# ahcorde/visualSLAM_Android

Hardware: AMD Instinct MI355X
Metric: frames/sec (TrackFrame+local BA) on 640×480 synthetic, 1/2/4/8 GPU (higher is better)
Workload: dtype f64

## Files before the change

### visualslam_android_amd/csrc/track.hip

```cpp
#include "vslam_internal.h"
#include "patch_dev.h"
#include "pvs_perm.h"

#define TRK_THREADS 256
#define SORT_CAP 4096
static_assert(SORT_CAP == PVS_SORT_CAP, "a level's list (at most max_points entries) fits the permutation's sort buffer");

template <class T>
DEVFN bool td_project(T& td, int& flags, const double* pos, const Pose& pose, const CamModel& cam, CamProj& pr) {
  flags &= ~TDF_IN_IMAGE;
  double c[3];
  pose_xform(pose, pos, c);
  td.cam[0] = c[0]; td.cam[1] = c[1]; td.cam[2] = c[2];
  if (c[2] < 0.001) return false;
  const double implane[2] = {c[0] / c[2], c[1] / c[2]};
  if (implane[0] * implane[0] + implane[1] * implane[1] > cam.largest_radius * cam.largest_radius) return false;
  pr = cam_project(cam, implane[0], implane[1]);
  td.image[0] = pr.im[0]; td.image[1] = pr.im[1];
  if (pr.invalid) return true;
  if (td.image[0] < 0 || td.image[1] < 0 || td.image[0] > cam.size[0] || td.image[1] > cam.size[1]) return true;
  flags |= TDF_IN_IMAGE;
  return true;
}

// ... 552 lines not shown
  }
  h00 = grp_sum<G>(h00); h01 = grp_sum<G>(h01); h02 = grp_sum<G>(h02);
  h11 = grp_sum<G>(h11); h12 = grp_sum<G>(h12); h22 = grp_sum<G>(h22);
  const double H[9] = {h00, h01, h02, h01, h11, h12, h02, h12, h22};
  double Hinv[9];
  inv3(H, Hinv);
  double sub0 = td.vfound[0], sub1 = td.vfound[1], meanDiff = 0.0;
  bool running = dosub, converged = false;
  for (int it = 0; __any(running); it++) {
    if (it >= nSubPixIts) running = false;
    double cx = 0, cy = 0;
    if (running) {
      cx = level_n_pos(sub0, level); cy = level_n_pos(sub1, level);
      const int xb = (int)(cx > 0.0 ? cx + 0.5 : cx - 0.5), yb = (int)(cy > 0.0 ? cy + 0.5 : cy - 0.5);
      const int b = HALF + 1;
      if (!(xb >= b && yb >= b && xb < cols - b && yb < rows - b)) running = false;
    }
    double p0[Q], p1[Q], p2[Q];
#pragma unroll
    for (int x = 0; x < Q; x++) { p0[x] = 0; p1[x] = 0; p2[x] = 0; }
    if (running && rowok) {
      const double bx = cx - HALF, by = cy - HALF;
      const double dX = bx - floor(bx), dY = by - floor(by);
      const float fTL = (float)((1.0 - dX) * (1.0 - dY)), fTR = (float)((dX) * (1.0 - dY));
      const float fBL = (float)((1.0 - dX) * (dY)), fBR = (float)((dX) * (dY));
      const uint8_t* r0 = img + (size_t)((int)by + sub) * ip + (int)bx + 1;
      const PRow<PS> q0 = load_row<PS>(r0), q1 = load_row<PS>(r0 + ip);
#pragma unroll
      for (int x = 1; x <= Q; x++) {
        const float fPixel = fTL * row_byte(q0, x - 1) + fTR * row_byte(q0, x) + fBL * row_byte(q1, x - 1) + fBR * row_byte(q1, x);
        const double dDiff = (fPixel - (float)row_byte(trow, x)) + meanDiff;
        p0[x - 1] = dDiff * gx[x - 1]; p1[x - 1] = dDiff * gy[x - 1]; p2[x - 1] = dDiff;
      }
    }
    double a0 = 0, a1 = 0, a2 = 0;
#pragma unroll 1
    for (int y = 1; y <= Q; y++) {
      if (sub == y) {
#pragma unroll
        for (int x = 0; x < Q; x++) { a0 += p0[x]; a1 += p1[x]; a2 += p2[x]; }
      }
      const int src = grp * G + y;
      a0 = __shfl(a0, src); a1 = __shfl(a1, src); a2 = __shfl(a2, src);
    }
    if (running) {
      const double u0 = Hinv[0] * a0 + Hinv[1] * a1 + Hinv[2] * a2;
      const double u1 = Hinv[3] * a0 + Hinv[4] * a1 + Hinv[5] * a2;
      const double u2 = Hinv[6] * a0 + Hinv[7] * a1 + Hinv[8] * a2;
      sub0 -= u0 * scale; sub1 -= u1 * scale; meanDiff -= u2;
      if (u0 * u0 + u1 * u1 < 0.03 * 0.03) { converged = true; running = false; }
    }
  }
  if (dosub && lead) {
    if (!converged) tdflags = flags & ~TDF_FOUND;
    else { td.vfound[0] = sub0; td.vfound[1] = sub1; }
  }
  for (int l = 0; l < NLEV; l++) {
    const int c = __popcll(__ballot(dosub && converged && lead && level == l));
    if (lane == 0 && c) atomicAdd(&st->found[l], c);
  }
}

#define SUBPIX_GRID 16
template <int PS, int G>
__global__ __launch_bounds__(64) void k_subpixN(MapDev m, TrackParams tp, SearchArgs a, int stage) {
  int s, bx;
  xcd_stream_block(a.nblk, a.S, s, bx);
  if (s < 0) return;
  TrackerState* st = &m.st[s];
  if (!trk_runs_track_map(m.held, s, st)) return;
  const int nsub = stage == 0 ? st->n_search : st->n_l3;
  for (int blk = bx; blk * (64 / G) < nsub; blk += a.nblk) subpix_block<PS, G>(m, tp, a, st, s, nsub, blk);
}

#define POSE_THREADS 128
#ifdef VSLAM_BA_PROF
__device__ unsigned long long g_pose_prof[16];
#define POSE_STAMP(id) do { if (blockIdx.x == 0 && threadIdx.x == 0) { const unsigned long long t_ = clock64(); g_pose_prof[id] += t_ - g_pose_prof[15]; g_pose_prof[15] = t_; } } while (0)
#else
#define POSE_STAMP(id) do { } while (0)
#endif
#define POSE_WAVES (POSE_THREADS / 64)
#ifndef POSE_ILP
#define POSE_ILP 2
#endif

struct PoseItem {
  double cam[3], image[2], derivs[4], vfound[2], sqrt_inv_noise;
  int flags, idx;
};
struct PoseWs { double* d; int* i; int P; };

DEVFN void item_load(PoseItem& it, const PoseWs& w, int e) {
  it.flags = w.i[e]; it.idx = w.i[w.P + e];
#pragma unroll
  for (int i = 0; i < 3; i++) it.cam[i] = w.d[(0 + i) * w.P + e];
#pragma unroll
  for (int i = 0; i < 2; i++) { it.image[i] = w.d[(3 + i) * w.P + e]; it.vfound[i] = w.d[(9 + i) * w.P + e]; }
#pragma unroll
  for (int i = 0; i < 4; i++) it.derivs[i] = w.d[(5 + i) * w.P + e];
  it.sqrt_inv_noise = w.d[11 * w.P + e];
}
DEVFN void item_store(const PoseItem& it, const PoseWs& w, int e, bool all) {
#pragma unroll
  for (int i = 0; i < 2; i++) w.d[(3 + i) * w.P + e] = it.image[i];
  if (!all) return;
  w.i[e] = it.flags;
#pragma unroll
  for (int i = 0; i < 3; i++) w.d[(0 + i) * w.P + e] = it.cam[i];
#pragma unroll
  for (int i = 0; i < 4; i++) w.d[(5 + i) * w.P + e] = it.derivs[i];
}

#define POSE_CHUNK 32
#define POSE_ENT 27
#define POSE_GRP 8
static_assert(2 * 2 * POSE_CHUNK * POSE_ENT + 2 * POSE_GRP * POSE_ENT + 64 <= SORT_CAP, "two record buffers (and the chain's two groups of read-ahead) in the sort buffer");
static_assert(POSE_THREADS == 128 && POSE_CHUNK == 32 && POSE_GRP % 2 == 0, "wavefront 0 chains, wavefront 1 produces");
static_assert(POSE_THREADS == VSLAM_POSE_WG && SORT_CAP == VSLAM_SELECT_LDS_CAP, "vslam_eval_select / vslam_eval_pose_tail run k_pose's workgroup");

DEVFN void pose_chain_load(double (&v)[POSE_GRP], const double __attribute__((address_space(3)))* p) {
#pragma unroll
  for (int u = 0; u < POSE_GRP; u++) v[u] = p[u * POSE_ENT];
}
DEVFN void pose_chain_add(double& acc, const double (&v)[POSE_GRP]) {
#pragma unroll
  for (int u = 0; u < POSE_GRP; u++) acc += v[u];
}

#ifdef VSLAM_BA_PROF
#define POSE_ACC_PROF_DECL unsigned long long tw_ = 0, tb_ = 0, tl_ = clock64()
#define POSE_ACC_BARRIER() do { const unsigned long long a_ = clock64(); tw_ += a_ - tl_; __syncthreads(); tl_ = clock64(); tb_ += tl_ - a_; } while (0)
#define POSE_ACC_PROF_END() do { if (blockIdx.x == 0 && (threadIdx.x & 63) == 0) { g_pose_prof[10 + 2 * (threadIdx.x >> 6)] += tw_; g_pose_prof[11 + 2 * (threadIdx.x >> 6)] += tb_; } } while (0)
#else
#define POSE_ACC_PROF_DECL do { } while (0)
#define POSE_ACC_BARRIER() __syncthreads()
#define POSE_ACC_PROF_END() do { } while (0)
#endif
#define PAS1 __attribute__((address_space(1)))
#define PAS3 __attribute__((address_space(3)))
__device__ __attribute__((noinline)) double pose_accumulate(const double PAS1* wd, int P, int nf, double wls_prior, bool qint, double sigma2, double PAS3* sortbuf) {
  const int lane = threadIdx.x & 63;
  nf = __builtin_amdgcn_readfirstlane(nf); P = __builtin_amdgcn_readfirstlane(P);
  const int nchunks = (nf + POSE_CHUNK - 1) / POSE_CHUNK;
  constexpr int BUF = 2 * POSE_CHUNK * POSE_ENT;
  POSE_ACC_PROF_DECL;
  double acc = 0.0;
  if (lane == 0 || lane == 6 || lane == 11 || lane == 15 || lane == 18 || lane == 20) acc = 0.0 + wls_prior;
  if (__builtin_amdgcn_readfirstlane(threadIdx.x >> 6) == 1) {
    const int row = lane & 1, pm = lane >> 1;
    struct Item { double cam[3], image[2], vfound[2], da, db, sqrt_inv_noise; };
#define POSE_ITEM_LOADS 10
    auto gld = [&](double& dst, int comp, int e) { asm volatile("global_load_dwordx2 %0, %1, off" : "=v"(dst) : "v"(wd + (size_t)comp * P + e)); };
    auto load_chunk = [&](Item& t, int k) {
      int e = k * POSE_CHUNK + pm;
      e = e < nf ? e : nf - 1;
#pragma unroll
      for (int i = 0; i < 3; i++) gld(t.cam[i], i, e);
#pragma unroll
      for (int i = 0; i < 2; i++) { gld(t.image[i], 3 + i, e); gld(t.vfound[i], 9 + i, e); }
      gld(t.da, 5 + 2 * row, e); gld(t.db, 6 + 2 * row, e);
      gld(t.sqrt_inv_noise, 11, e);
    };
#define POSE_WAIT_SET(t, N) asm volatile("s_waitcnt vmcnt(" #N ")" : "+v"(t.cam[0]), "+v"(t.cam[1]), "+v"(t.cam[2]), "+v"(t.image[0]), "+v"(t.image[1]), \
                                         "+v"(t.vfound[0]), "+v"(t.vfound[1]), "+v"(t.da), "+v"(t.db), "+v"(t.sqrt_inv_noise))
    auto produce = [&](const Item& t, int e, double PAS3* buf) {
      double PAS3* dst = buf + lane * POSE_ENT;
      double w = 0.0, err[2] = {0.0, 0.0};
      if (e < nf) {
        err[0] = (t.vfound[0] - t.image[0]) * t.sqrt_inv_noise; err[1] = (t.vfound[1] - t.image[1]) * t.sqrt_inv_noise;
        const double es = err[0] * err[0] + err[1] * err[1];
        w = tukey_weight(es, sigma2);
      }
      if (w == 0.0) {
#pragma unroll
        for (int k = 0; k < POSE_ENT; k++) dst[k] = 0.0;
        return;
      }
      const double ooz = 1.0 / t.cam[2];
      const double c[3] = {t.cam[0], t.cam[1], t.cam[2]};
      double J[6], wJ[6];
#pragma unroll
      for (int m = 0; m < 6; m++) {
        double f0, f1;
        se3_generator_motion(m, c, ooz, f0, f1);
        J[m] = t.sqrt_inv_noise * (t.da * f0 + t.db * f1);
        wJ[m] = w * J[m];
      }
      const double e_ = row ? err[1] : err[0];
      const double mm = qint ? (double)(int)e_ : e_;
      int q = 0;
#pragma unroll
      for (int r = 0; r < 6; r++)
#pragma unroll
        for (int cc = r; cc < 6; cc++) dst[q++] = wJ[r] * J[cc];
#pragma unroll
      for (int k = 0; k < 6; k++) dst[21 + k] = mm * wJ[k];
    };
    Item it0, it1, it2;
    load_chunk(it0, 0); load_chunk(it1, 1); load_chunk(it2, 2);
    POSE_ACC_BARRIER();
    POSE_WAIT_SET(it0, 20);
    produce(it0, pm, sortbuf);
    POSE_ACC_BARRIER();
    auto prod_step = [&](int k, Item& tprod, Item& tload) {
      if (k + 1 < nchunks) {
        load_chunk(tload, k + 3);
        POSE_WAIT_SET(tprod, 20);
        produce(tprod, (k + 1) * POSE_CHUNK + pm, sortbuf + ((k + 1) & 1) * BUF);
      }
      POSE_ACC_BARRIER();
    };
    for (int k = 0; k < nchunks; k += 3) {
      prod_step(k, it1, it0);
      if (k + 1 < nchunks) prod_step(k + 1, it2, it1);
      if (k + 2 < nchunks) prod_step(k + 2, it0, it2);
    }
    asm volatile("s_waitcnt vmcnt(0)" ::: "memory");
  } else {
    POSE_ACC_BARRIER();
    POSE_ACC_BARRIER();
    for (int k = 0; k < nchunks; k++) {
      const int left = nf - k * POSE_CHUNK;
      const int ng = (2 * (left < POSE_CHUNK ? left : POSE_CHUNK) + POSE_GRP - 1) / POSE_GRP;
      constexpr int GSTR = POSE_GRP * POSE_ENT;
      const double PAS3* rp = sortbuf + (k & 1) * BUF + lane;
      double x0[POSE_GRP], x1[POSE_GRP], x2[POSE_GRP];
      pose_chain_load(x0, rp);
      pose_chain_load(x1, rp + GSTR);
      for (int g = 0; g < ng; g += 3) {
        pose_chain_load(x2, rp + (g + 2) * GSTR);
        __builtin_amdgcn_sched_barrier(0);
        pose_chain_add(acc, x0);
        __builtin_amdgcn_sched_barrier(0);
        if (g + 1 >= ng) break;
        pose_chain_load(x0, rp + (g + 3) * GSTR);
        __builtin_amdgcn_sched_barrier(0);
        pose_chain_add(acc, x1);
        __builtin_amdgcn_sched_barrier(0);
        if (g + 2 >= ng) break;
        pose_chain_load(x1, rp + (g + 4) * GSTR);
        __builtin_amdgcn_sched_barrier(0);
        pose_chain_add(acc, x2);
        __builtin_amdgcn_sched_barrier(0);
      }
      POSE_ACC_BARRIER();
    }
  }
  POSE_ACC_PROF_END();
  return acc;
}

__device__ __attribute__((noinline)) void pose_tail(double acc, double PAS3* pose, double PAS3* up) {
  double mu[6];
  wave_pose_solve(acc, mu);
  POSE_STAMP(6);
  wave_pose_apply(mu, pose);
  if ((threadIdx.x & 63) == 0) {
#pragma unroll
    for (int r = 0; r < 6; r++) up[r] = mu[r];
  }
}

DEVFN void calc_pose_update(const PoseWs& ws, MapPointDev* pts, int nf, const TrackParams& tp,
                            double dOverrideSigma, bool bMarkOutliers, double* sortbuf, Pose* pose ,
                            double* up , int* hist , unsigned long long* sel , const unsigned* selmm ) {
  const bool wave0 = __builtin_amdgcn_readfirstlane(threadIdx.x >> 6) == 0;
  if (nf == 0) {
    if (wave0) pose_tail(0.0, (double PAS3*)(double*)pose, (double PAS3*)up);
    __syncthreads();
    return;
  }
  POSE_STAMP(2);
  double sigma2;
  if (dOverrideSigma > 0) sigma2 = dOverrideSigma;
  else {
    const double med = block_radix_select(sortbuf, nf, nf / 2, hist, sel, selmm);
    sigma2 = tukey_sigma_squared(med, (unsigned long)nf);
  }
  POSE_STAMP(3);
  const double acc = pose_accumulate((const double PAS1*)ws.d, ws.P, nf, tp.wls_prior, (tp.quirks & VSLAM_Q_POSE_INT_RESIDUAL) != 0, sigma2, (double PAS3*)sortbuf);
  if (bMarkOutliers) {
    for (int e = threadIdx.x; e < nf; e += POSE_THREADS) {
      const double sn = ws.d[11 * ws.P + e];
      const double e0 = (ws.d[9 * ws.P + e] - ws.d[3 * ws.P + e]) * sn, e1 = (ws.d[10 * ws.P + e] - ws.d[4 * ws.P + e]) * sn;
      MapPointDev* mp = pts + ws.i[ws.P + e];
      if (tukey_weight(e0 * e0 + e1 * e1, sigma2) == 0.0) mp->n_out++; else mp->n_in++;
    }
  }
  POSE_STAMP(4);
  if (wave0) pose_tail(acc, (double PAS3*)(double*)pose, (double PAS3*)up);
  __syncthreads();
}

#ifndef VSLAM_POSE_WAVES
#define VSLAM_POSE_WAVES 2
#endif
__global__ __launch_bounds__(POSE_THREADS) __attribute__((amdgpu_waves_per_eu(VSLAM_POSE_WAVES, VSLAM_POSE_WAVES))) void k_pose(MapDev m, TrackParams tp, int stage) {
  const int s = blockIdx.x;
  TrackerState* st = &m.st[s];
  if (!trk_runs_track_map(m.held, s, st)) return;
  const int P = tp.max_points;
  TrackData* td = m.td + (size_t)s * P;
  MapPointDev* pts = m.pts + (size_t)s * P;
  const int* ilist = m.iter_list + (size_t)s * P;
  __shared__ double sortbuf[SORT_CAP];
  __shared__ double red[2];
  __shared__ double last_up[6];
  __shared__ int gcnt[4 * POSE_WAVES];
  __shared__ __attribute__((aligned(16))) int hist[768];
  __shared__ unsigned long long sel[1];
  __shared__ unsigned selmm[2 * POSE_WAVES];
  __shared__ Pose pose;
  if (threadIdx.x == 0) pose = st->pose_cur;
  if (threadIdx.x < 6) last_up[threadIdx.x] = 0.0;
  const int n = stage == 0 ? st->n_coarse : st->n_iter;
  if (stage == 0) {
    if (n == 0) return;
    const int nFound = st->found[0] + st->found[1] + st->found[2] + st->found[3];
    if (nFound < tp.coarse_min) return;
  }
#ifdef VSLAM_BA_PROF
  if (blockIdx.x == 0 && threadIdx.x == 0) g_pose_prof[15] = clock64();
#endif
  const PoseWs ws = {m.pose_ws + (size_t)s * POSE_WS_COMPS * P, m.pose_wsi + (size_t)s * 2 * P, P};
  const int lane = threadIdx.x & 63, wave = threadIdx.x >> 6;
  constexpr int POSE_GB = 4;
  int nf = 0;
  for (int e0 = 0; e0 < n; e0 += POSE_GB * POSE_THREADS) {
    int idx[POSE_GB], fl[POSE_GB]; bool fnd[POSE_GB]; unsigned long long bm[POSE_GB]; double v[POSE_GB][12];
#pragma unroll
    for (int u = 0; u < POSE_GB; u++) { const int e = e0 + u * POSE_THREADS + threadIdx.x; idx[u] = ilist[e < n ? e : n - 1]; }
#pragma unroll
    for (int u = 0; u < POSE_GB; u++) {
      const int e = e0 + u * POSE_THREADS + threadIdx.x;
      fl[u] = m.pt_flags[(size_t)s * P + idx[u]];
      fnd[u] = e < n && (fl[u] & TDF_FOUND);
    }
#pragma unroll
    for (int u = 0; u < POSE_GB; u++) {
      const TrackData& t = td[idx[u]];
      for (int i = 0; i < 3; i++) v[u][i] = t.cam[i];
      for (int i = 0; i < 2; i++) { v[u][3 + i] = t.image[i]; v[u][9 + i] = t.vfound[i]; }
      for (int i = 0; i < 4; i++) v[u][5 + i] = t.derivs[i];
      v[u][11] = t.sqrt_inv_noise;
    }
#pragma unroll
    for (int u = 0; u < POSE_GB; u++) { bm[u] = __ballot(fnd[u]); if (lane == 0) gcnt[u * POSE_WAVES + wave] = __popcll(bm[u]); }
    __syncthreads();
#pragma unroll
    for (int u = 0; u < POSE_GB; u++) {
      int off = nf;
      for (int w = 0; w < POSE_WAVES; w++) { const int c = gcnt[u * POSE_WAVES + w]; if (w < wave) off += c; nf += c; }
      if (!fnd[u]) continue;
      const int f = off + __popcll(bm[u] & ((1ull << lane) - 1ull));
      ws.i[f] = fl[u]; ws.i[P + f] = idx[u];
#pragma unroll
      for (int c = 0; c < 12; c++) ws.d[c * P + f] = v[u][c];
    }
    __syncthreads();
  }
  POSE_STAMP(0);
  for (int iter = 0; iter < 10; iter++) {
    const bool nonlinear = stage == 0 || iter == 0 || iter == 4 || iter == 9;
    SelectRange sr = select_range_empty();
    for (int e0 = threadIdx.x; e0 < nf; e0 += POSE_ILP * POSE_THREADS) {
      PoseItem t[POSE_ILP]; double pos[POSE_ILP][3];
#pragma unroll
      for (int u = 0; u < POSE_ILP; u++) {
        const int e = e0 + u * POSE_THREADS;
        item_load(t[u], ws, e < nf ? e : nf - 1);
      }
      if (nonlinear && iter != 0) {
#pragma unroll
        for (int u = 0; u < POSE_ILP; u++)
#pragma unroll
          for (int k = 0; k < 3; k++) pos[u][k] = pts[t[u].idx].pos[k];
      }
#pragma unroll
      for (int u = 0; u < POSE_ILP; u++) {
        const int e = e0 + u * POSE_THREADS;
        if (e >= nf) continue;
        if (iter != 0) {
          if (nonlinear) td_project_and_derivs(t[u], t[u].flags, pos[u], pose, tp.cam);
          else {
            double jac[12], a = 0, b = 0;
            td_calc_jacobian(t[u], jac);
#pragma unroll
            for (int k = 0; k < 6; k++) { a += jac[k] * last_up[k]; b += jac[6 + k] * last_up[k]; }
            t[u].image[0] += a; t[u].image[1] += b;
          }
          item_store(t[u], ws, e, nonlinear);
        }
        const double r0 = (t[u].vfound[0] - t[u].image[0]) * t[u].sqrt_inv_noise;
        const double r1 = (t[u].vfound[1] - t[u].image[1]) * t[u].sqrt_inv_noise;
        const double e2 = r0 * r0 + r1 * r1;
        sortbuf[e] = e2;
        select_range_add(sr, e2);
      }
    }
    block_select_publish(sr, hist, selmm);
    __syncthreads();
    POSE_STAMP(1);
    const double override_sigma = iter > 5 ? (stage == 0 ? 1.0 : 16.0) : 0.0;
    calc_pose_update(ws, pts, nf, tp, override_sigma, stage == 1 && iter == 9, sortbuf, &pose, last_up, hist, sel, selmm);
    POSE_STAMP(7);
  }
  POSE_STAMP(8);
  MeasDev* cm = m.cur_meas + (size_t)s * P;
  if (stage != 0) {
    for (int i = threadIdx.x; i < st->n_points; i += POSE_THREADS) cm[i].valid = 0;
    __syncthreads();
  }
  for (int e0 = threadIdx.x; e0 < nf; e0 += POSE_GB * POSE_THREADS) {
    int idx[POSE_GB], fl[POSE_GB], lv[POSE_GB]; double v[POSE_GB][11];
#pragma unroll
    for (int u = 0; u < POSE_GB; u++) {
      const int e = e0 + u * POSE_THREADS, ec = e < nf ? e : nf - 1;
      idx[u] = ws.i[P + ec]; fl[u] = ws.i[ec];
#pragma unroll
      for (int c = 0; c < 11; c++) v[u][c] = ws.d[c * P + ec];
    }
    if (stage != 0) {
#pragma unroll
      for (int u = 0; u < POSE_GB; u++) lv[u] = m.pt_level[(size_t)s * P + idx[u]];
    }
#pragma unroll
    for (int u = 0; u < POSE_GB; u++) {
      const int e = e0 + u * POSE_THREADS;
      if (e >= nf) continue;
      TrackData& t = td[idx[u]];
      m.pt_flags[(size_t)s * P + idx[u]] = fl[u];
      for (int i = 0; i < 3; i++) t.cam[i] = v[u][i];
      for (int i = 0; i < 2; i++) t.image[i] = v[u][3 + i];
      for (int i = 0; i < 4; i++) t.derivs[i] = v[u][5 + i];
      if (stage != 0) {
        MeasDev mm;
        mm.root[0] = v[u][9]; mm.root[1] = v[u][10];
        mm.valid = 1; mm.level = (signed char)lv[u]; mm.subpix = (fl[u] & TDF_SUBPIX) ? 1 : 0; mm.source = 0 ; mm.pad = 0;
        cm[idx[u]] = mm;
        sortbuf[e] = v[u][2];
      }
    }
  }
  if (stage == 0) {
    if (threadIdx.x == 0) { st->pose_cur = pose; st->did_coarse = 1; }
    return;
  }
  __syncthreads();
  if (threadIdx.x < 2) {
    double a = 0.0;
    const bool sq = threadIdx.x == 1;
    int k = 0;
    for (; k + 8 <= nf; k += 8) {
      double z[8];
#pragma unroll
      for (int u = 0; u < 8; u++) z[u] = sortbuf[k + u];
#pragma unroll
      for (int u = 0; u < 8; u++) a += sq ? z[u] * z[u] : z[u];
    }
    for (; k < nf; k++) { const double z = sortbuf[k]; a += sq ? z * z : z; }
    red[threadIdx.x] = a;
  }
  __syncthreads();
  if (threadIdx.x != 0) return;
  const double dSum = red[0], dSumSq = red[1];
  const int nNum = nf;
  if (nNum > 20) {
    st->depth_mean = dSum / nNum;
    st->depth_sigma = sqrt((dSumSq / nNum) - (st->depth_mean) * (st->depth_mean));
  }
  st->pose_cur = pose; st->pose_final = pose;
  const bool recovered = st->recovered_now != 0;
  st->recovered_now = 0;
  if (!recovered) {
    const Pose nfo = pose_mul(pose, pose_inverse(st->start_pose));
    double motion[6];
    se3_ln(nfo, motion);
    double ss = 0;
    for (int i = 0; i < 6; i++) {
      st->velocity[i] = 0.9 * (0.5 * motion[i] + 0.5 * st->velocity[i]);
      double v = st->velocity[i];
      if (i < 3) v *= 1.0 / st->depth_mean;
      ss += v * v;
    }
    st->msd_vel = sqrt(ss);
  }
  const Pose* kfp = m.kf_pose + (size_t)s * tp.max_keyframes;
  double closest = 9999999999.9;
  for (int k = 0; k < st->n_kf; k++) { const double d = kf_linear_dist(pose, kfp[k]); if (d < closest) closest = d; }
  {
    int ta = 0, tf = 0, la = 0, lf = 0;
    for (int i = 0; i < NLEV; i++) { ta += st->attempted[i]; tf += st->found[i]; if (i >= 2) { la += st->attempted[i]; lf += st->found[i]; } }
    int quality;
    if (tf == 0 || ta == 0) quality = 0;
    else {
      const double dTotal = (double)tf / ta;
      const double dLarge = la > 10 ? (double)lf / la : dTotal;
      if (dTotal > 0.3) quality = 2; else if (dLarge < 0.13) quality = 0; else quality = 1;
    }
    if (quality == 1 && closest > tp.wiggle_scale * 10.0) quality = 0;
    if (quality == 0) st->lost_frames++; else st->lost_frames = 0;
    st->quality = quality;
  }
  if (!recovered) {
    double dDist = closest;
    dDist *= (1.0 / st->depth_mean);
    const bool need = dDist > tp.max_kf_dist_wiggle_mult * st->wiggle_depth_norm;
    if (st->quality == 2 && need && st->frame - st->last_kf_dropped > tp.min_frames_between_kf &&
        (st->n_kf < tp.max_keyframes || (tp.keyframe_retire && st->ba_countdown <= 0))) {
      st->kf_pending = 1;
      st->last_kf_dropped = st->frame;
    }
  }
  POSE_STAMP(9);
}

#ifdef VSLAM_BA_PROF
extern "C" int vslam_debug_search_prof(unsigned long long* out, int reset) {
  HIPCHK(hipDeviceSynchronize());
  HIPCHK(hipMemcpyFromSymbol(out, HIP_SYMBOL(g_search_prof), sizeof(unsigned long long) * 2 * SEARCH_PROF_SLOTS));
  if (reset) { unsigned long long z[2 * SEARCH_PROF_SLOTS] = {0}; HIPCHK(hipMemcpyToSymbol(HIP_SYMBOL(g_search_prof), z, sizeof(z))); }
  out[15] = SEARCH_N; out[SEARCH_PROF_SLOTS + 15] = SEARCH_K;
  return VSLAM_OK;
}
extern "C" int vslam_debug_pose_prof(unsigned long long* out16, int reset) {
  HIPCHK(hipDeviceSynchronize());
  HIPCHK(hipMemcpyFromSymbol(out16, HIP_SYMBOL(g_pose_prof), sizeof(unsigned long long) * 16));
  if (reset) { unsigned long long z[16] = {0}; HIPCHK(hipMemcpyToSymbol(HIP_SYMBOL(g_pose_prof), z, sizeof(z))); }
  return VSLAM_OK;
}
#endif

int trk_alloc(vslam_system* sys) {
  const vslam_params& p = sys->p;
  const size_t S = sys->S, P = p.max_points, K = p.max_keyframes;
  if (P > SORT_CAP) { vslam_set_error("max_points %d exceeds %d", (int)P, SORT_CAP); return VSLAM_E_INVALID; }
  MapDev& m = sys->map; DevOwner& own = sys->own; hipStream_t q = sys->stream;
  VCHK(own.alloc(&m.pts, S * P, q)); VCHK(own.alloc(&m.td, S * P, q)); VCHK(own.alloc(&m.tmpl, S * P * TMPL_PITCH, q));
  VCHK(own.alloc(&m.kf_meas, S * K * P, q)); VCHK(own.alloc(&m.cur_meas, S * P, q));
  VCHK(own.alloc(&m.kf_pose, S * K, q)); VCHK(own.alloc(&m.kf_fixed, S * K, q)); VCHK(own.alloc(&m.kf_depth, S * K * 2, q));
  for (int l = 0; l < NLEV; l++) VCHK(own.alloc(&m.kf_img[l], S * K * (size_t)sys->geom[l].pitch * sys->geom[l].h, q));
  VCHK(own.alloc(&m.st, S, q)); VCHK(own.alloc(&m.pvs_list, S * NLEV * P, q)); VCHK(own.alloc(&m.search_list, S * P, q)); VCHK(own.alloc(&m.iter_list, S * P, q)); VCHK(own.alloc(&m.pt_level, S * P, q)); VCHK(own.alloc(&m.pt_flags, S * P, q));
  VCHK(own.alloc(&m.pose_ws, S * POSE_WS_COMPS * P, q)); VCHK(own.alloc(&m.pose_wsi, S * 2 * P, q));
  trk_fill_params(p, sys->tp);
  return VSLAM_OK;
}

void cam_fill(CamModel& c, const double cam5[5], double width, double height, int quirks) {
  c.size[0] = width; c.size[1] = height;
  c.focal[0] = c.size[0] * cam5[0]; c.focal[1] = c.size[1] * cam5[1];
  c.center[0] = c.size[0] * cam5[2] - 0.5; c.center[1] = c.size[1] * cam5[3] - 0.5;
  c.w = cam5[4];
  double one_over_2tan = 0;
  if (c.w != 0.0) { c.two_tan = 2.0 * vlm::vtan(c.w / 2.0); one_over_2tan = 1.0 / c.two_tan; c.winv = 1.0 / c.w; c.distortion_enabled = 1.0; }
  else { c.winv = 0; c.two_tan = 0; c.distortion_enabled = 0; }
  double v2[2];
  if (quirks & VSLAM_Q_CAM_INT_RADIUS) {
    int m1 = (int)cam5[2], m2 = (int)(1.0 - cam5[2]);
    v2[0] = (m1 > m2 ? m1 : m2) / cam5[0];
    m1 = (int)cam5[3]; m2 = (int)(1.0 - cam5[3]);
    v2[1] = (m1 > m2 ? m1 : m2) / cam5[1];
  } else {
    v2[0] = (cam5[2] > 1.0 - cam5[2] ? cam5[2] : 1.0 - cam5[2]) / cam5[0];
    v2[1] = (cam5[3] > 1.0 - cam5[3] ? cam5[3] : 1.0 - cam5[3]) / cam5[1];
  }
  const double rr = sqrt(v2[0] * v2[0] + v2[1] * v2[1]);
  c.largest_radius = c.w == 0.0 ? rr : vlm::vtan(rr * c.w) * one_over_2tan;
  c.max_r = 1.5 * c.largest_radius;
}

void trk_fill_params(const vslam_params& p, TrackParams& t) {
  cam_fill(t.cam, p.cam, p.width, p.height, p.quirks);
  t.P = p.patch_size; t.max_ssd = 500 * p.patch_size * p.patch_size;
  t.max_patches = p.max_patches_per_frame; t.coarse_min = p.coarse_min; t.coarse_max = p.coarse_max; t.coarse_range = p.coarse_range;
  t.coarse_subpix_its = p.coarse_subpix_its; t.coarse_disabled = p.coarse_disabled; t.fine_subpix_its = p.fine_subpix_its;
  t.coarse_min_vel = p.coarse_min_vel; t.wls_prior = p.wls_prior;
  t.min_frames_between_kf = p.min_frames_between_kf; t.max_kf_dist_wiggle_mult = p.max_kf_dist_wiggle_mult; t.wiggle_scale = p.wiggle_scale;
  t.ba_max_iterations = p.ba_max_iterations; t.ba_convergence_limit = p.ba_convergence_limit;
  t.ba_min_sigma2 = p.ba_min_tukey_sigma * p.ba_min_tukey_sigma; t.ba_window = p.ba_window; t.ba_min_keyframes = p.ba_min_keyframes;
  t.quirks = p.quirks; t.max_points = p.max_points; t.max_keyframes = p.max_keyframes; t.ba_delay = p.ba_delay_frames;
  t.ba_batch = p.ba_batch_frames > 1 ? p.ba_batch_frames : 1;
  t.ba_sum_order = p.ba_sum_order ? 1 : 0;
  t.grow_map = p.grow_map;
  t.idle = p.idle_iterations != 0; t.fq_cap = 8192;
  t.keyframe_retire = p.keyframe_retire ? 1 : 0;
  {
    double a[2], b[2];
    cam_unproject(t.cam, t.cam.size[0] / 2, t.cam.size[1] / 2, a);
    cam_unproject(t.cam, t.cam.size[0] / 2 + 1, t.cam.size[1] / 2 + 1, b);
    const double d0 = a[0] - b[0], d1 = a[1] - b[1];
    t.one_pixel_dist = sqrt(d0 * d0 + d1 * d1) / sqrt(2.0);
  }
  const int kcap_max[NLEV] = {16384, 8192, 4096, 2048};
  for (int l = 0; l < NLEV; l++) t.kcap[l] = p.max_corners[l] < kcap_max[l] ? p.max_corners[l] : kcap_max[l];

}

static void trk_search_args(vslam_system* sys, SearchArgs& a) {
  for (int l = 0; l < NLEV; l++) {
    a.img[l] = sys->fr.img[l]; a.img_sstride[l] = sys->fr.img_sstride[l]; a.img_pitch[l] = sys->fr.img_pitch[l];
    a.corners[l] = sys->fr.corners[l]; a.rowlut[l] = sys->fr.rowlut[l];
    a.w[l] = sys->geom[l].w; a.h[l] = sys->geom[l].h; a.cap[l] = sys->geom[l].cap;
    a.kf_pitch[l] = sys->geom[l].pitch; a.kf_stride[l] = (size_t)sys->geom[l].pitch * sys->geom[l].h;
  }
  a.ncorners = sys->fr.ncorners;
}

typedef void (*PlanKernel)(MapDev, TrackParams, int);
static PlanKernel plan_kernel(const vslam_system* sys) { return sys->p.pvs_shuffle_seed ? k_plan<true> : k_plan<false>; }

int trk_search_stage(vslam_system* sys, int stage) {
  const int S = sys->S, P = sys->p.max_points;
  MapDev& m = sys->map;
  const TrackParams& tp = sys->tp;
  SearchArgs a;
  trk_search_args(sys, a);
  a.S = S; a.nblk = 1;
  if (stage == 0) {
    prof_mark(sys, PROF_PVS);
    overlay_note_track_map(sys);
    hipLaunchKernelGGL(k_motion, dim3((S + 63) / 64), dim3(64), 0, sys->stream, m, S, sys->p.use_sbi ? (const double*)sys->fr.sbi_rot : (const double*)nullptr);
    hipLaunchKernelGGL(k_pvs, dim3((P + TRK_THREADS - 1) / TRK_THREADS, S), dim3(TRK_THREADS), 0, sys->stream, m, tp);
    prof_mark(sys, PROF_PLAN_COARSE);
    hipLaunchKernelGGL(plan_kernel(sys), dim3(S), dim3(TRK_THREADS), 0, sys->stream, m, tp, 0);
    prof_mark(sys, PROF_SEARCH_COARSE);
    if (!tp.coarse_disabled || sys->p.relocalise) {
// ... 94 lines not shown
```

### visualslam_android_amd/csrc/vslam_internal.h

```cpp
#pragma once
#include <hip/hip_runtime.h>
#include <stdint.h>
#include <string>
#include <vector>
#include "../../include/vslam_c.h"
#include "dev_math.h"

#define NLEV VSLAM_LEVELS

void vslam_set_error(const char* fmt, ...);

#define HIPCHK(expr)                                                                         \
  do {                                                                                       \
    hipError_t _e = (expr);                                                                  \
    if (_e != hipSuccess) {                                                                  \
      vslam_set_error("%s:%d: %s -> %s", __FILE__, __LINE__, #expr, hipGetErrorString(_e)); \
      return VSLAM_E_HIP;                                                                    \
    }                                                                                        \
  } while (0)

#define VCHK(expr) do { int _r = (expr); if (_r) return _r; } while (0)

static inline Pose pose_from12(const double* q) { Pose p; for (int i = 0; i < 9; i++) p.R[i] = q[i]; for (int i = 0; i < 3; i++) p.t[i] = q[9 + i]; return p; }
static inline void pose_to12(const Pose& p, double* q) { for (int i = 0; i < 9; i++) q[i] = p.R[i]; for (int i = 0; i < 3; i++) q[9 + i] = p.t[i]; }

struct LevelGeom {
  int w, h;
  int pitch;
  int nchunk;
  int cap;
  int thr;
};

struct FrameDev {
  const uint8_t* img[NLEV];
  size_t img_sstride[NLEV];
  int img_pitch[NLEV];
  unsigned long long* cmask[NLEV];
  int* rowcnt[NLEV];
  int* rowlut[NLEV];
  uint32_t* corners[NLEV];
  int* ncorners;
  int* overflow;
  int* scores[NLEV];
  uint32_t* maxcorners[NLEV];
  int* nmax;
  uint8_t* sbi_small;
  float* sbi_tmpl;
  float* sbi_jacs;
  double* sbi_rot;
  int* step_list;
  unsigned char* held;
};


#define POSE_WS_COMPS 12
#define TMPL_PITCH 128

struct MapPointDev {
  double pos[3], right[3], down[3];
  int src_kf, src_level, irx, iry;
  int bad, n_in, n_out, n_meas_kfs;
};

#define TDF_IN_IMAGE 1
#define TDF_FOUND 2
#define TDF_SEARCHED 4
#define TDF_SUBPIX 8
#define TDF_TMPL_BAD 16
#define TDF_HAVE_LAST 32

struct TrackData {
  double cam[3], image[2], derivs[4];
  double vfound[2], sqrt_inv_noise;
  double warp_inv[4], last_warp[4];
  int tsum, tsumsq;
};

struct MeasDev {
  double root[2];
  signed char valid, level, subpix, source;
  int pad;
};

#define BOOT_MAX_TRAILS 1000

struct TrackerState {
  Pose pose_final, start_pose, pose_cur;
  double velocity[6];
  double msd_vel, depth_mean, depth_sigma, wiggle_depth_norm;
  int frame, last_kf_dropped, lost_frames, quality;
  int attempted[NLEV], found[NLEV];
  int did_coarse, just_recovered, map_good, kf_pending;
  int n_points, n_kf;
  int pvs_count[NLEV], pvs_head[NLEV];
  int n_coarse, n_search, n_iter, n_l3;
  int coarse_range, fine_range, coarse_found;
  int ba_accepted, kf_added, ba_converged_recent, ba_converged_full;
  int ba_countdown;
  unsigned long long n_zmssd, n_ba_trials;
  int newq_head;
  int fq_n;
  int idle_count;
  int idle_do_fail;
  int n_refound_new, n_refound_failed, n_ba_all, n_ba_recent_idle;
  int init_stage;
  int spacebar;
  int n_trails, trail_buf;
  int boot_action;
  int boot_run;
  int boot_ok, n_hom_inliers, n_init_points;
  unsigned boot_seed;
  int boot_host_matches;
  int recovered_now;
  unsigned pvs_seed;
};
HDFN void tracker_reset_fields(TrackerState& st, unsigned pvs_seed) {
  st.boot_seed = 1u; st.pvs_seed = pvs_seed;
  st.quality = 2; st.last_kf_dropped = -20; st.depth_mean = 1.0; st.depth_sigma = 1.0;
  st.ba_accepted = -2; st.ba_countdown = -1;
  st.ba_converged_recent = 1; st.ba_converged_full = 1;
  for (int i = 0; i < 9; i++) st.pose_final.R[i] = (i % 4 == 0) ? 1.0 : 0.0;
  st.pose_cur = st.pose_final; st.start_pose = st.pose_final;
}
HDFN TrackerState tracker_reset_state(unsigned pvs_seed) { TrackerState st = {}; tracker_reset_fields(st, pvs_seed); return st; }
DEVFN bool trk_in_step(const unsigned char* held, int s) { return !held || !held[s]; }
DEVFN bool trk_runs_track_map(const unsigned char* held, int s, const TrackerState* st) {
  return trk_in_step(held, s) && st->map_good && (st->lost_frames < 3 || st->recovered_now);
}
DEVFN bool trk_kf_pending(const unsigned char* held, int s, const TrackerState* st) { return trk_in_step(held, s) && st->kf_pending; }

struct TrackParams {
  CamModel cam;
  int P;
  int max_ssd;
  int max_patches, coarse_min, coarse_max, coarse_range, coarse_subpix_its, coarse_disabled, fine_subpix_its;
  double coarse_min_vel, wls_prior;
  int min_frames_between_kf; double max_kf_dist_wiggle_mult, wiggle_scale;
  int ba_max_iterations; double ba_convergence_limit, ba_min_sigma2; int ba_window, ba_min_keyframes;
// ... 344 lines not shown
```

Baseline: 535,500.

## Stage point positions and levels in pose workspace; fold iteration-0 residuals into gather

The pose kernel now copies each found point's 3D position and pyramid level into extra workspace planes during the initial gather, so the iterative loop no longer does indirect loads through the map point array. Iteration-0 residuals and select range are computed during the gather, and the per-iteration step is split into templated linear/nonlinear variants with higher ILP and gather batch. The tail reads tracker state up front and computes the closest-keyframe distance in parallel on one wavefront, instead of a serial loop on a single thread. It costs more workspace memory and registers, which could hurt occupancy.

```diff
diff --git a/visualslam_android_amd/csrc/track.hip b/visualslam_android_amd/csrc/track.hip
--- a/visualslam_android_amd/csrc/track.hip
+++ b/visualslam_android_amd/csrc/track.hip
@@ -658,34 +658,43 @@
 #endif
 #define POSE_WAVES (POSE_THREADS / 64)
 #ifndef POSE_ILP
-#define POSE_ILP 2
+#define POSE_ILP 4
 #endif
-
+#ifndef POSE_GB
+#define POSE_GB 8
+#endif
+#define PAS1 __attribute__((address_space(1)))
+#define PAS3 __attribute__((address_space(3)))
+
+#define POSE_WS_POS 12
+static_assert(POSE_WS_COMPS == POSE_WS_POS + 3 && POSE_WSI_PLANES == 3, "k_pose's working set: 12 tracker doubles + the position; flags, index, level");
 struct PoseItem {
   double cam[3], image[2], derivs[4], vfound[2], sqrt_inv_noise;
-  int flags, idx;
+  int flags;
 };
 struct PoseWs { double* d; int* i; int P; };
 
-DEVFN void item_load(PoseItem& it, const PoseWs& w, int e) {
-  it.flags = w.i[e]; it.idx = w.i[w.P + e];
-#pragma unroll
-  for (int i = 0; i < 3; i++) it.cam[i] = w.d[(0 + i) * w.P + e];
-#pragma unroll
-  for (int i = 0; i < 2; i++) { it.image[i] = w.d[(3 + i) * w.P + e]; it.vfound[i] = w.d[(9 + i) * w.P + e]; }
-#pragma unroll
-  for (int i = 0; i < 4; i++) it.derivs[i] = w.d[(5 + i) * w.P + e];
-  it.sqrt_inv_noise = w.d[11 * w.P + e];
-}
-DEVFN void item_store(const PoseItem& it, const PoseWs& w, int e, bool all) {
-#pragma unroll
-  for (int i = 0; i < 2; i++) w.d[(3 + i) * w.P + e] = it.image[i];
-  if (!all) return;
-  w.i[e] = it.flags;
-#pragma unroll
-  for (int i = 0; i < 3; i++) w.d[(0 + i) * w.P + e] = it.cam[i];
-#pragma unroll
-  for (int i = 0; i < 4; i++) w.d[(5 + i) * w.P + e] = it.derivs[i];
+template <bool ALL>
+DEVFN void item_load(PoseItem& it, const double PAS1* wd, const int PAS1* wi, int P, int e) {
+  if (ALL) it.flags = wi[e];
+#pragma unroll
+  for (int i = 0; i < 3; i++) it.cam[i] = wd[(0 + i) * P + e];
+#pragma unroll
+  for (int i = 0; i < 2; i++) { it.image[i] = wd[(3 + i) * P + e]; it.vfound[i] = wd[(9 + i) * P + e]; }
+#pragma unroll
+  for (int i = 0; i < 4; i++) it.derivs[i] = wd[(5 + i) * P + e];
+  it.sqrt_inv_noise = wd[11 * P + e];
+}
+template <bool ALL>
+DEVFN void item_store(const PoseItem& it, double PAS1* wd, int PAS1* wi, int P, int e) {
+#pragma unroll
+  for (int i = 0; i < 2; i++) wd[(3 + i) * P + e] = it.image[i];
+  if (!ALL) return;
+  wi[e] = it.flags;
+#pragma unroll
+  for (int i = 0; i < 3; i++) wd[(0 + i) * P + e] = it.cam[i];
+#pragma unroll
+  for (int i = 0; i < 4; i++) wd[(5 + i) * P + e] = it.derivs[i];
 }
 
 #define POSE_CHUNK 32
@@ -713,8 +722,6 @@
 #define POSE_ACC_BARRIER() __syncthreads()
 #define POSE_ACC_PROF_END() do { } while (0)
 #endif
-#define PAS1 __attribute__((address_space(1)))
-#define PAS3 __attribute__((address_space(3)))
 __device__ __attribute__((noinline)) double pose_accumulate(const double PAS1* wd, int P, int nf, double wls_prior, bool qint, double sigma2, double PAS3* sortbuf) {
   const int lane = threadIdx.x & 63;
   nf = __builtin_amdgcn_readfirstlane(nf); P = __builtin_amdgcn_readfirstlane(P);
@@ -838,6 +845,43 @@
   }
 }
 
+template <bool NONLINEAR>
+DEVFN SelectRange pose_step_trips(double PAS1* wd, int PAS1* wi, int P, int nf, const Pose& pose, const double* last_up, const CamModel& cam, double PAS3* sortbuf) {
+  SelectRange sr = select_range_empty();
+  for (int e0 = threadIdx.x; e0 < nf; e0 += POSE_ILP * POSE_THREADS) {
+    PoseItem t[POSE_ILP]; double pos[POSE_ILP][3];
+#pragma unroll
+    for (int u = 0; u < POSE_ILP; u++) {
+      const int e = e0 + u * POSE_THREADS, ec = e < nf ? e : nf - 1;
+      item_load<NONLINEAR>(t[u], wd, wi, P, ec);
+      if (NONLINEAR) {
+#pragma unroll
+        for (int k = 0; k < 3; k++) pos[u][k] = wd[(POSE_WS_POS + k) * P + ec];
+      }
+    }
+#pragma unroll
+    for (int u = 0; u < POSE_ILP; u++) {
+      const int e = e0 + u * POSE_THREADS;
+      if (e >= nf) continue;
+      if (NONLINEAR) td_project_and_derivs(t[u], t[u].flags, pos[u], pose, cam);
+      else {
+        double jac[12], a = 0, b = 0;
+        td_calc_jacobian(t[u], jac);
+#pragma unroll
+        for (int k = 0; k < 6; k++) { a += jac[k] * last_up[k]; b += jac[6 + k] * last_up[k]; }
+        t[u].image[0] += a; t[u].image[1] += b;
+      }
+      item_store<NONLINEAR>(t[u], wd, wi, P, e);
+      const double r0 = (t[u].vfound[0] - t[u].image[0]) * t[u].sqrt_inv_noise;
+      const double r1 = (t[u].vfound[1] - t[u].image[1]) * t[u].sqrt_inv_noise;
+      const double e2 = r0 * r0 + r1 * r1;
+      sortbuf[e] = e2;
+      select_range_add(sr, e2);
+    }
+  }
+  return sr;
+}
+
 DEVFN void calc_pose_update(const PoseWs& ws, MapPointDev* pts, int nf, const TrackParams& tp,
                             double dOverrideSigma, bool bMarkOutliers, double* sortbuf, Pose* pose ,
                             double* up , int* hist , unsigned long long* sel , const unsigned* selmm ) {
@@ -881,9 +925,9 @@
   MapPointDev* pts = m.pts + (size_t)s * P;
   const int* ilist = m.iter_list + (size_t)s * P;
   __shared__ double sortbuf[SORT_CAP];
-  __shared__ double red[2];
+  __shared__ double red[3];
   __shared__ double last_up[6];
-  __shared__ int gcnt[4 * POSE_WAVES];
+  __shared__ int gcnt[POSE_GB * POSE_WAVES];
   __shared__ __attribute__((aligned(16))) int hist[768];
   __shared__ unsigned long long sel[1];
   __shared__ unsigned selmm[2 * POSE_WAVES];
@@ -899,22 +943,18 @@
 #ifdef VSLAM_BA_PROF
   if (blockIdx.x == 0 && threadIdx.x == 0) g_pose_prof[15] = clock64();
 #endif
-  const PoseWs ws = {m.pose_ws + (size_t)s * POSE_WS_COMPS * P, m.pose_wsi + (size_t)s * 2 * P, P};
+  const PoseWs ws = {m.pose_ws + (size_t)s * POSE_WS_COMPS * P, m.pose_wsi + (size_t)s * POSE_WSI_PLANES * P, P};
   const int lane = threadIdx.x & 63, wave = threadIdx.x >> 6;
-  constexpr int POSE_GB = 4;
   int nf = 0;
+  SelectRange sr = select_range_empty();
   for (int e0 = 0; e0 < n; e0 += POSE_GB * POSE_THREADS) {
-    int idx[POSE_GB], fl[POSE_GB]; bool fnd[POSE_GB]; unsigned long long bm[POSE_GB]; double v[POSE_GB][12];
+    int idx[POSE_GB], fl[POSE_GB], lv[POSE_GB], f[POSE_GB]; unsigned long long bm[POSE_GB]; double v[POSE_GB][12];
 #pragma unroll
     for (int u = 0; u < POSE_GB; u++) { const int e = e0 + u * POSE_THREADS + threadIdx.x; idx[u] = ilist[e < n ? e : n - 1]; }
 #pragma unroll
     for (int u = 0; u < POSE_GB; u++) {
-      const int e = e0 + u * POSE_THREADS + threadIdx.x;
       fl[u] = m.pt_flags[(size_t)s * P + idx[u]];
-      fnd[u] = e < n && (fl[u] & TDF_FOUND);
-    }
-#pragma unroll
-    for (int u = 0; u < POSE_GB; u++) {
+      lv[u] = m.pt_level[(size_t)s * P + idx[u]];
       const TrackData& t = td[idx[u]];
       for (int i = 0; i < 3; i++) v[u][i] = t.cam[i];
       for (int i = 0; i < 2; i++) { v[u][3 + i] = t.image[i]; v[u][9 + i] = t.vfound[i]; }
@@ -922,61 +962,52 @@
       v[u][11] = t.sqrt_inv_noise;
     }
 #pragma unroll
-    for (int u = 0; u < POSE_GB; u++) { bm[u] = __ballot(fnd[u]); if (lane == 0) gcnt[u * POSE_WAVES + wave] = __popcll(bm[u]); }
+    for (int u = 0; u < POSE_GB; u++) {
+      const int e = e0 + u * POSE_THREADS + threadIdx.x;
+      const bool fnd = e < n && (fl[u] & TDF_FOUND);
+      bm[u] = __ballot(fnd); f[u] = fnd ? 0 : -1;
+      if (lane == 0) gcnt[u * POSE_WAVES + wave] = __popcll(bm[u]);
+    }
     __syncthreads();
 #pragma unroll
     for (int u = 0; u < POSE_GB; u++) {
       int off = nf;
       for (int w = 0; w < POSE_WAVES; w++) { const int c = gcnt[u * POSE_WAVES + w]; if (w < wave) off += c; nf += c; }
-      if (!fnd[u]) continue;
-      const int f = off + __popcll(bm[u] & ((1ull << lane) - 1ull));
-      ws.i[f] = fl[u]; ws.i[P + f] = idx[u];
-#pragma unroll
-      for (int c = 0; c < 12; c++) ws.d[c * P + f] = v[u][c];
+      if (f[u] < 0) continue;
+      f[u] = off + __popcll(bm[u] & ((1ull << lane) - 1ull));
+      ws.i[f[u]] = fl[u]; ws.i[P + f[u]] = idx[u]; ws.i[2 * P + f[u]] = lv[u];
+#pragma unroll
+      for (int c = 0; c < 12; c++) ws.d[c * P + f[u]] = v[u][c];
+      const double r0 = (v[u][9] - v[u][3]) * v[u][11];
+      const double r1 = (v[u][10] - v[u][4]) * v[u][11];
+      const double e2 = r0 * r0 + r1 * r1;
+      sortbuf[f[u]] = e2;
+      select_range_add(sr, e2);
+    }
+    double pos[POSE_GB][3];
+#pragma unroll
+    for (int u = 0; u < POSE_GB; u++)
+#pragma unroll
+      for (int k = 0; k < 3; k++) pos[u][k] = pts[idx[u]].pos[k];
+#pragma unroll
+    for (int u = 0; u < POSE_GB; u++) {
+      if (f[u] < 0) continue;
+#pragma unroll
+      for (int k = 0; k < 3; k++) ws.d[(POSE_WS_POS + k) * P + f[u]] = pos[u][k];
     }
     __syncthreads();
   }
+  block_select_publish(sr, hist, selmm);
+  __syncthreads();
   POSE_STAMP(0);
   for (int iter = 0; iter < 10; iter++) {
-    const bool nonlinear = stage == 0 || iter == 0 || iter == 4 || iter == 9;
-    SelectRange sr = select_range_empty();
-    for (int e0 = threadIdx.x; e0 < nf; e0 += POSE_ILP * POSE_THREADS) {
-      PoseItem t[POSE_ILP]; double pos[POSE_ILP][3];
-#pragma unroll
-      for (int u = 0; u < POSE_ILP; u++) {
-        const int e = e0 + u * POSE_THREADS;
-        item_load(t[u], ws, e < nf ? e : nf - 1);
-      }
-      if (nonlinear && iter != 0) {
-#pragma unroll
-        for (int u = 0; u < POSE_ILP; u++)
-#pragma unroll
-          for (int k = 0; k < 3; k++) pos[u][k] = pts[t[u].idx].pos[k];
-      }
-#pragma unroll
-      for (int u = 0; u < POSE_ILP; u++) {
-        const int e = e0 + u * POSE_THREADS;
-        if (e >= nf) continue;
-        if (iter != 0) {
-          if (nonlinear) td_project_and_derivs(t[u], t[u].flags, pos[u], pose, tp.cam);
-          else {
-            double jac[12], a = 0, b = 0;
-            td_calc_jacobian(t[u], jac);
-#pragma unroll
-            for (int k = 0; k < 6; k++) { a += jac[k] * last_up[k]; b += jac[6 + k] * last_up[k]; }
-            t[u].image[0] += a; t[u].image[1] += b;
-          }
-          item_store(t[u], ws, e, nonlinear);
-        }
-        const double r0 = (t[u].vfound[0] - t[u].image[0]) * t[u].sqrt_inv_noise;
-        const double r1 = (t[u].vfound[1] - t[u].image[1]) * t[u].sqrt_inv_noise;
-        const double e2 = r0 * r0 + r1 * r1;
-        sortbuf[e] = e2;
-        select_range_add(sr, e2);
-      }
-    }
-    block_select_publish(sr, hist, selmm);
-    __syncthreads();
+    if (iter != 0) {
+      const bool nonlinear = stage == 0 || iter == 4 || iter == 9;
+      if (nonlinear) sr = pose_step_trips<true>((double PAS1*)ws.d, (int PAS1*)ws.i, P, nf, pose, last_up, tp.cam, (double PAS3*)sortbuf);
+      else sr = pose_step_trips<false>((double PAS1*)ws.d, (int PAS1*)ws.i, P, nf, pose, last_up, tp.cam, (double PAS3*)sortbuf);
+      block_select_publish(sr, hist, selmm);
+      __syncthreads();
+    }
     POSE_STAMP(1);
     const double override_sigma = iter > 5 ? (stage == 0 ? 1.0 : 16.0) : 0.0;
     calc_pose_update(ws, pts, nf, tp, override_sigma, stage == 1 && iter == 9, sortbuf, &pose, last_up, hist, sel, selmm);
@@ -993,13 +1024,9 @@
 #pragma unroll
     for (int u = 0; u < POSE_GB; u++) {
       const int e = e0 + u * POSE_THREADS, ec = e < nf ? e : nf - 1;
-      idx[u] = ws.i[P + ec]; fl[u] = ws.i[ec];
+      idx[u] = ws.i[P + ec]; fl[u] = ws.i[ec]; lv[u] = ws.i[2 * P + ec];
 #pragma unroll
       for (int c = 0; c < 11; c++) v[u][c] = ws.d[c * P + ec];
-    }
-    if (stage != 0) {
-#pragma unroll
-      for (int u = 0; u < POSE_GB; u++) lv[u] = m.pt_level[(size_t)s * P + idx[u]];
     }
 #pragma unroll
     for (int u = 0; u < POSE_GB; u++) {
@@ -1024,6 +1051,25 @@
     return;
   }
   __syncthreads();
+  const int n_kf = st->n_kf;
+  double depth_mean = 0, wiggle_depth_norm = 0, vel[6] = {0, 0, 0, 0, 0, 0};
+  int recovered_now = 0, att[NLEV] = {0, 0, 0, 0}, fnd[NLEV] = {0, 0, 0, 0}, lost_frames = 0, frame = 0, last_kf_dropped = 0, ba_countdown = 0;
+  Pose start_pose;
+  if (threadIdx.x == 0) {
+    depth_mean = st->depth_mean; wiggle_depth_norm = st->wiggle_depth_norm; recovered_now = st->recovered_now;
+    for (int i = 0; i < 6; i++) vel[i] = st->velocity[i];
+    for (int i = 0; i < NLEV; i++) { att[i] = st->attempted[i]; fnd[i] = st->found[i]; }
+    lost_frames = st->lost_frames; frame = st->frame; last_kf_dropped = st->last_kf_dropped; ba_countdown = st->ba_countdown;
+    start_pose = st->start_pose;
+  }
+  if (wave == POSE_WAVES - 1) {
+    const Pose* kfp = m.kf_pose + (size_t)s * tp.max_keyframes;
+    double closest = 9999999999.9;
+    for (int k = lane; k < n_kf; k += 64) { const double d = kf_linear_dist(pose, kfp[k]); if (d < closest) closest = d; }
+#pragma unroll
+    for (int o = 32; o >= 1; o >>= 1) { const double d = __shfl_xor(closest, o); if (d < closest) closest = d; }
+    if (lane == 0) red[2] = closest;
+  }
   if (threadIdx.x < 2) {
     double a = 0.0;
     const bool sq = threadIdx.x == 1;
@@ -1040,35 +1086,33 @@
   }
   __syncthreads();
   if (threadIdx.x != 0) return;
-  const double dSum = red[0], dSumSq = red[1];
+  const double dSum = red[0], dSumSq = red[1], closest = red[2];
   const int nNum = nf;
   if (nNum > 20) {
-    st->depth_mean = dSum / nNum;
-    st->depth_sigma = sqrt((dSumSq / nNum) - (st->depth_mean) * (st->depth_mean));
+    depth_mean = dSum / nNum;
+    st->depth_mean = depth_mean;
+    st->depth_sigma = sqrt((dSumSq / nNum) - (depth_mean) * (depth_mean));
   }
   st->pose_cur = pose; st->pose_final = pose;
-  const bool recovered = st->recovered_now != 0;
+  const bool recovered = recovered_now != 0;
   st->recovered_now = 0;
   if (!recovered) {
-    const Pose nfo = pose_mul(pose, pose_inverse(st->start_pose));
+    const Pose nfo = pose_mul(pose, pose_inverse(start_pose));
     double motion[6];
     se3_ln(nfo, motion);
     double ss = 0;
     for (int i = 0; i < 6; i++) {
-      st->velocity[i] = 0.9 * (0.5 * motion[i] + 0.5 * st->velocity[i]);
-      double v = st->velocity[i];
-      if (i < 3) v *= 1.0 / st->depth_mean;
+      double v = 0.9 * (0.5 * motion[i] + 0.5 * vel[i]);
+      st->velocity[i] = v;
+      if (i < 3) v *= 1.0 / depth_mean;
       ss += v * v;
     }
     st->msd_vel = sqrt(ss);
   }
-  const Pose* kfp = m.kf_pose + (size_t)s * tp.max_keyframes;
-  double closest = 9999999999.9;
-  for (int k = 0; k < st->n_kf; k++) { const double d = kf_linear_dist(pose, kfp[k]); if (d < closest) closest = d; }
+  int quality;
   {
     int ta = 0, tf = 0, la = 0, lf = 0;
-    for (int i = 0; i < NLEV; i++) { ta += st->attempted[i]; tf += st->found[i]; if (i >= 2) { la += st->attempted[i]; lf += st->found[i]; } }
-    int quality;
+    for (int i = 0; i < NLEV; i++) { ta += att[i]; tf += fnd[i]; if (i >= 2) { la += att[i]; lf += fnd[i]; } }
     if (tf == 0 || ta == 0) quality = 0;
     else {
       const double dTotal = (double)tf / ta;
@@ -1076,17 +1120,17 @@
       if (dTotal > 0.3) quality = 2; else if (dLarge < 0.13) quality = 0; else quality = 1;
     }
     if (quality == 1 && closest > tp.wiggle_scale * 10.0) quality = 0;
-    if (quality == 0) st->lost_frames++; else st->lost_frames = 0;
+    st->lost_frames = quality == 0 ? lost_frames + 1 : 0;
     st->quality = quality;
   }
   if (!recovered) {
     double dDist = closest;
-    dDist *= (1.0 / st->depth_mean);
-    const bool need = dDist > tp.max_kf_dist_wiggle_mult * st->wiggle_depth_norm;
-    if (st->quality == 2 && need && st->frame - st->last_kf_dropped > tp.min_frames_between_kf &&
-        (st->n_kf < tp.max_keyframes || (tp.keyframe_retire && st->ba_countdown <= 0))) {
+    dDist *= (1.0 / depth_mean);
+    const bool need = dDist > tp.max_kf_dist_wiggle_mult * wiggle_depth_norm;
+    if (quality == 2 && need && frame - last_kf_dropped > tp.min_frames_between_kf &&
+        (n_kf < tp.max_keyframes || (tp.keyframe_retire && ba_countdown <= 0))) {
       st->kf_pending = 1;
-      st->last_kf_dropped = st->frame;
+      st->last_kf_dropped = frame;
     }
   }
   POSE_STAMP(9);
@@ -1118,7 +1162,7 @@
   VCHK(own.alloc(&m.kf_pose, S * K, q)); VCHK(own.alloc(&m.kf_fixed, S * K, q)); VCHK(own.alloc(&m.kf_depth, S * K * 2, q));
   for (int l = 0; l < NLEV; l++) VCHK(own.alloc(&m.kf_img[l], S * K * (size_t)sys->geom[l].pitch * sys->geom[l].h, q));
   VCHK(own.alloc(&m.st, S, q)); VCHK(own.alloc(&m.pvs_list, S * NLEV * P, q)); VCHK(own.alloc(&m.search_list, S * P, q)); VCHK(own.alloc(&m.iter_list, S * P, q)); VCHK(own.alloc(&m.pt_level, S * P, q)); VCHK(own.alloc(&m.pt_flags, S * P, q));
-  VCHK(own.alloc(&m.pose_ws, S * POSE_WS_COMPS * P, q)); VCHK(own.alloc(&m.pose_wsi, S * 2 * P, q));
+  VCHK(own.alloc(&m.pose_ws, S * POSE_WS_COMPS * P, q)); VCHK(own.alloc(&m.pose_wsi, S * POSE_WSI_PLANES * P, q));
   trk_fill_params(p, sys->tp);
   return VSLAM_OK;
 }
diff --git a/visualslam_android_amd/csrc/vslam_internal.h b/visualslam_android_amd/csrc/vslam_internal.h
--- a/visualslam_android_amd/csrc/vslam_internal.h
+++ b/visualslam_android_amd/csrc/vslam_internal.h
@@ -54,7 +54,8 @@
 };
 
 
-#define POSE_WS_COMPS 12
+#define POSE_WS_COMPS 15
+#define POSE_WSI_PLANES 3
 #define TMPL_PITCH 128
 
 struct MapPointDev {
```

New measurement: 541,900 (median of 6 runs). No clear change (+1.2%).
